# ogotoh/spaln

Hardware: AMD Instinct MI355X
Metric: GCUPS (DP cell updates/s), cDNA->genome spliced DP (higher is better)
Workload: dtype f32 (exact integers) / int32; 1 GPU; C2: 10k x 2 kb cDNA vs planted loci +-1 kb (windows ~12 kb), default band, Fwd2s1 _wip path: alignS_ng(ori=1, -Q0) = UDH sweep + slab tracebacks, SKL out; queries_per_gpu=10000, queries_total=10000, parallelism=1 rank(s), one per GPU, queries sharded, no collective on the data path

## Files before the change

### include/spdp.h

```cpp
#ifndef SPDP_H_
#define SPDP_H_

#include <stdint.h>
#include <stddef.h>

#ifdef __cplusplus
extern "C" {
#endif

#define SPDP_MAX_QUANT   8
#define SPDP_NEVSEL      (INT32_MIN / 16 * 7)
#define SPDP_END_OF_ULK  (INT32_MAX - 2)
#define SPDP_REF_NELEM   16

typedef struct SpdpScoring {
    int32_t mtx_dim;
    int32_t mtx[32 * 32];
    int32_t gop, gep;
    int32_t lgop, lgep;
    int32_t noll;
    int32_t spj;
    int32_t llmt;
    int32_t ipen;
    int32_t nquant;
// ... 129 lines not shown
typedef struct SpdpHspSource {
    void* user;
    int  (*units)(void* user, int32_t query, int32_t level, const int32_t span[8], const int32_t** flat, int32_t* n_flat);
    void (*release)(void* user, int32_t query, const int32_t* flat);
} SpdpHspSource;
int spdp_align_s_seeded(SpdpContext* ctx, const SpdpScoring* sc, const SpdpSeedParams* sp,
                        const SpdpProblem* probs, int n_probs, const SpdpJuxt* const* hsps, const int32_t* n_hsps,
                        const int32_t* lowest_level, const SpdpHspSource* src, SpdpAlignment* out);
int spdp_align_s_seeded_ori3(SpdpContext* ctx, const SpdpScoring* sc, const SpdpSeedParams* sp,
                             const SpdpProblem* fwd, const SpdpProblem* rev, int n_probs,
                             const SpdpJuxt* const* hsps, const int32_t* n_hsps, const int32_t* lowest_level,
                             const SpdpHspSource* src, SpdpAlignment* out, int32_t* orient);
int spdp_seeded_stats(const SpdpContext* ctx, int64_t* out, int n);
void spdp_rerun_stats(SpdpContext* ctx, int64_t* out, int reset);
void spdp_sweep_stats(SpdpContext* ctx, int64_t out[4], int reset);

int spdp_corner_list(const SpdpSkl* recs, int n, int m_unit, SpdpSkl* out);

typedef struct SpdpExon {
    int32_t left, right;
    int32_t rleft, rright;
    int32_t mch, mmc, gap, unp;
    int32_t mch5, mmc5, gap5, unp5;
    int32_t mch3, mmc3, gap3, unp3;
    int32_t phs;
    int32_t escr, iscr;
    int32_t sig3, sig5;
} SpdpExon;

typedef struct SpdpRescoreParams {
// ... 436 lines not shown
```

### spaln_amd/csrc/spdp_api.cpp

```cpp

#include <hip/hip_runtime.h>
#include <algorithm>
#include <cstdio>
#include <cstdlib>
#include <cstring>
#include <atomic>
#include <string>
#include <thread>
#include <vector>

#include "../../include/spdp.h"
#include "spdp_dev.h"
#include "spdp_internal.h"

static void stripe_rng(int a_left, int a_right, int b_left, int b_right, int sh, SpdpWindow* w)
{
    if (sh < 0) {
        int shorter = std::min(a_right - a_left, b_right - b_left);
        sh = -sh * shorter / 100;
    }
    w->up = b_right - a_right;
    w->lw = b_left - a_left;
    if (w->up < w->lw) std::swap(w->up, w->lw);
    w->up += sh;
// ... 117 lines not shown
        SpdpContext* l = spdp_create(ctx->device);
        if (!l) return nullptr;
        ctx->lanes.push_back(l);
    }
    return ctx->lanes[i - 1];
}

void spdp_destroy(SpdpContext* ctx)
{
    if (!ctx) return;
    for (SpdpContext* l : ctx->lanes) spdp_destroy(l);
    ctx->lanes.clear();
    (void) hipSetDevice(ctx->device);
    for (DevPool& p : ctx->pool) p.release();
    for (int k = 0; k < 3; ++k) if (ctx->stage_ptr[k]) (void) hipHostFree(ctx->stage_ptr[k]);
    (void) hipEventDestroy(ctx->ev0);
    (void) hipEventDestroy(ctx->ev1);
    (void) hipEventDestroy(ctx->ev2);
    (void) hipEventDestroy(ctx->ev3);
    if (ctx->stream2) (void) hipStreamDestroy(ctx->stream2);
    (void) hipStreamDestroy(ctx->stream);
    delete ctx;
}

void* SpdpContext::staging(int k, size_t bytes)
{
    if (bytes <= stage_cap[k]) return stage_ptr[k];
    if (stage_ptr[k]) (void) hipHostFree(stage_ptr[k]);
    stage_ptr[k] = nullptr; stage_cap[k] = 0;
    const size_t want = bytes + bytes / 8;
    if (hipHostMalloc(&stage_ptr[k], want, hipHostMallocDefault) != hipSuccess) { stage_ptr[k] = nullptr; return nullptr; }
    stage_cap[k] = want;
    return stage_ptr[k];
}

int spdp_upload_ring(SpdpContext* ctx, const std::vector<int64_t>& off, int64_t tot, int64_t grp_positions,
                     std::vector<StagedStream>& st, const std::function<void(int i, int64_t at)>& pack)
// ... 533 lines not shown
    case BY_ROWWAVE_UDH: HIPCHK(spdp_launch_rowwave_udh(&S, strm())); break;
    default:             HIPCHK(spdp_launch_rowwave(cut ? 2 : T.arg, &S, strm())); break;
    }
    HIPCHK(hipEventRecord(eve(), strm()));
    return 0;
}

int DevRun::launch_sweep()
{
    const RunTraits& T = traits();
    SweepArgs A;
    A.sc = (const DevScoring*) store->d_sc; A.probs = (const DevProblem*) d_probs; A.n_probs = n;
    A.a_codes = (const uint8_t*) store->d_a; A.cols = (const int2*) store->d_cols; A.bnd = (int*) d_bnd;
    A.tb = (uint8_t*) d_tb; A.imd = (int*) d_imd; A.res = (DevResult*) d_res; A.n_multi = n_multi;
    A.cross_g = cross_g; A.gprog = (int*) d_gprog;
    int grid = cross_g > 0 ? n * cross_g : n_multi + (n - n_multi + wpb - 1) / wpb;
    if (cross_g > 0 && getenv("SPDP_CROSS_TEST_SHORT")) --grid;
    HIPCHK(hipEventRecord(evb(), strm()));
    const int nq = std::max(1, std::min(store->sc.nquant, SPDP_MAX_QUANT));
    const int pen_cap = nq > 1 ? store->sc.qm_len[nq - 2] + 1 : 0;
    bool done = false;
    if (fp_ok && (T.kind != KIND_FORWARD || spdp_knob_on("SPDP_FP_FWD")) && !store->sc.local) {
        const hipError_t e = spdp_launch_sweep_fp(T.arg, 0, store->sc.spj ? 1 : 0, nq, pen_cap, store->sc.llmt, &A, grid, wpb, strm());
        if (e == hipSuccess) done = true;
        else if (e != hipErrorNotSupported) HIPCHK(e);
    }
    if (!done) HIPCHK(spdp_launch_sweep(T.arg, store->sc.local ? 1 : 0, nq, pen_cap, &A, grid, wpb, strm()));
    ++ctx->sweep_stats[done ? 0 : 1];
    if (cross_g > 0) ++ctx->sweep_stats[2];
    if (wpb == 16) ++ctx->sweep_stats[3];
// ... 15 lines not shown
    if (reset) ctx->rerun_stats[0] = ctx->rerun_stats[1] = 0;
    for (SpdpContext* l : ctx->lanes) {
        out[0] += l->rerun_stats[0]; out[1] += l->rerun_stats[1];
        if (reset) l->rerun_stats[0] = l->rerun_stats[1] = 0;
    }
}

extern "C" void spdp_sweep_stats(SpdpContext* ctx, int64_t* out, int reset)
{
    if (!ctx || !out) return;
    for (int k = 0; k < 4; ++k) {
        out[k] = reset ? ctx->sweep_stats[k].exchange(0) : ctx->sweep_stats[k].load();
        for (SpdpContext* l : ctx->lanes)
            out[k] += reset ? l->sweep_stats[k].exchange(0) : l->sweep_stats[k].load();
    }
}

int DevRun::sync()
{
    HIPCHK(hipStreamSynchronize(strm()));
    in_flight = false;
    if (cross_g > 0) {
        const size_t per = (size_t) cross_g * wpb + 2;
        std::vector<int> words(per * n);
        HIPCHK(spdp_copy_sync(words.data(), d_gprog, sizeof(int) * words.size(), hipMemcpyDeviceToHost, strm()));
        bool gave_up = false;
        for (int j = 0; j < n; ++j) gave_up = gave_up || words[per * j + per - 1] != 0;
        if (gave_up) {
            ++ctx->rerun_stats[0];
            if (getenv("SPDP_TRACE_RUNS")) fprintf(stderr, "[spdp run] a cross-CU group was not resident%s: launch repeated without the groups\n", side ? " (side stream, beside another launch)" : "");
// ... 274 lines not shown
```

### spaln_amd/csrc/spdp_host.cpp

```cpp

#include <algorithm>
#include <cmath>
#include <cstdlib>
#include <cstring>
#include <vector>
#include <chrono>
#include <condition_variable>
#include <cstdio>
#include <mutex>
#include <thread>

#include "spdp_internal.h"

namespace {

const int kEndOfUlk = SPDP_END_OF_ULK;
const float kCoefB = 2.0f;
const int kScalarRows = 8;

struct Rng { int al, ar, bl, br; uint8_t a_exgl, a_exgr, b_exgl, b_exgr; };

struct Job {
    int score = SPDP_NEVSEL;
    bool score_set = false;
    bool failed = false;
    bool edge = false;
    std::vector<SpdpSkl> rec;
// ... 101 lines not shown
    if (s.size() >= 2) {
        const int i = s[1].m - s[0].m, j = s[1].n - s[0].n;
        if ((p.a_exgl && !i) || (p.b_exgl && !j)) s.erase(s.begin());
    }
    if (s.size() >= 2) {
        const size_t k = s.size() - 1;
        const int i = s[k].m - s[k - 1].m, j = s[k].n - s[k - 1].n;
        if ((p.a_exgr && !i) || (p.b_exgr && !j)) s.pop_back();
    }
}

}
void trim_skl_of(std::vector<SpdpSkl>& s, const SpdpProblem& p) { trim_skl(s, p); }
namespace {

struct ChunkGate {
    std::mutex m;
    std::condition_variable cv;
    int state = 0;
    hipEvent_t ev = nullptr;
    void open(int st_) { { std::lock_guard<std::mutex> g(m); if (state == 0) state = st_; } cv.notify_all(); }
    int wait() { std::unique_lock<std::mutex> g(m); cv.wait(g, [&] { return state != 0; }); return state; }
};

struct Aligner {
    SpdpContext* ctx;
    const DevStore* st;
    const SpdpProblem* probs;
    int n;
    int base = 0;
    ChunkGate* gate_in = nullptr;
    ChunkGate* gate_out = nullptr;
    SpdpAlignment* out = nullptr;
    bool raw = false;
    const SpdpRequests* req = nullptr;
    int parent(int job) const { return req ? req->parents[base + job] : base + job; }
    std::vector<TbItem> ctbs;
    std::vector<Job> jobs;
// ... 144 lines not shown
            trcbk(u.job, cur, w, false);
        }
    }

    double t_mark = 0;
    bool timing = getenv("SPDP_TIMING") != nullptr;
    void lap(const char* what)
    {
        if (!timing) return;
        const double now = std::chrono::duration<double, std::milli>(
            std::chrono::steady_clock::now().time_since_epoch()).count();
        if (t_mark > 0) fprintf(stderr, "[spdp timing] %-28s %8.2f ms\n", what, now - t_mark);
        t_mark = now;
    }

    int run()
    {
        const int rc = run_chunk();
        if (gate_out) gate_out->open(2);
        if (!rc && out) for (int i = 0; i < n; ++i) finish(i, out + i);
        return rc;
    }

    int run_chunk()
    {
        const SpdpScoring& sc = st->sc;
        lap("start");
        jobs.assign(n, Job());
        for (int i = 0; i < n; ++i) {
            const SpdpProblem& p = probs[i];
            Rng r{p.a_left, p.a_right, p.b_left, p.b_right, p.a_exgl, p.a_exgr, p.b_exgl, p.b_exgr};
            SpdpWindow w;
            stripe_of(r, sc.sh, &w);
            if (req) {
// ... 29 lines not shown
                if (side.build(st, items, RUN_WIP_FORWARD) || side.launch()) return -1;
                lap("side fwd build+launch");
            }
            may_overlap = false;
            if (udh.empty()) continue;
            std::vector<RunItem> items;
            for (const UdhItem& u : udh) {
                items.push_back(run_item(parent(u.job), u.r, u.w, u.n_imd));
                items.back().imd_intvl = u.imd_intvl;
            }
            DevRun run(ctx);
            run.beside = !side_tbs.empty();
            const bool a0 = sc.scalar_engines == 1;
            if (run.build(st, items, a0 ? RUN_A0_UDH : (sc.scalar_engines == 2 ? RUN_A1_UDH : RUN_WIP_UDH))) return -1;
            lap("udh build");
            if (first_round && gate_in && gate_in->wait() == 1) HIPCHK(hipStreamWaitEvent(run.strm(), gate_in->ev, 0));
            if (run.launch()) return -1;
            if (first_round && gate_out) {
                HIPCHK(hipEventRecord(gate_out->ev, run.strm()));
                gate_out->open(1);
            }
            first_round = false;
            if (run.sync()) return -1;
            lap("udh launch+sync");
            kernel_ms += run.kernel_ms; kernel_cells += run.total_cells;
            stats[0] += run.kernel_ms; stats[1] += (double) run.total_cells; stats[2] += (double) items.size();
            stats[6] += 1;
            std::vector<int32_t> scores, cpos, ranges;
            std::vector<int32_t> edge;
            if (run.fetch_udh(scores, cpos, ranges, &edge)) return -1;
            std::vector<DevResult> ures;
            if (a0 && run.fetch_results(ures)) return -1;
            lap("udh fetch");
            const int stride = run.cpos_stride();
            for (size_t k = 0; k < udh.size(); ++k) {
// ... 142 lines not shown
        memcpy(out->skl + 1, s.data(), sizeof(SpdpSkl) * s.size());
    }
};

}

struct SpdpBatch {
    SpdpContext* ctx = nullptr;
    DevStore store;
    std::vector<SpdpProblem> probs;
    DevRun score;
    bool score_built = false;
    double stats[SPDP_N_STATS] = {0};
};

SpdpBatch* spdp_batch_upload(SpdpContext* ctx, const SpdpScoring* sc, const SpdpProblem* probs, int n)
{
    if (!ctx || n <= 0) return nullptr;
    SpdpBatch* b = new SpdpBatch();
    b->ctx = ctx;
    b->probs.assign(probs, probs + n);
    if (b->store.upload(ctx, sc, probs, n)) { delete b; return nullptr; }
    return b;
}

void spdp_batch_free(SpdpBatch* bt) { delete bt; }

int64_t spdp_batch_cells(const SpdpBatch* bt)
{
    if (!bt) return 0;
// ... 17 lines not shown
    }
    if (bt->score.launch() || bt->score.sync()) return -1;
    if (kernel_ms) *kernel_ms = bt->score.kernel_ms;
    if (scores) {
        std::vector<DevResult> r;
        if (bt->score.fetch_results(r)) return -1;
        for (size_t i = 0; i < r.size(); ++i) scores[i] = r[i].score;
    }
    return 0;
}

static int align_on_store(SpdpContext* ctx, const DevStore* st, const SpdpProblem* probs, int n,
                          SpdpAlignment* out, float* kernel_ms, int64_t* kernel_cells,
                          double* stats = nullptr, bool raw = false, const SpdpRequests* req = nullptr)
{
    int n_chunks = n >= 4096 ? 2 : 1;
    if (const char* e = getenv("SPDP_CHUNKS")) n_chunks = std::max(1, std::min(atoi(e), 8));
    n_chunks = std::min(n_chunks, std::max(1, n / 64));
    if (req) n_chunks = 1;
    std::vector<Aligner> al(n_chunks);
    std::vector<ChunkGate> gates(n_chunks);
    std::vector<int> rc(n_chunks, 0);
    for (int c = 0; c < n_chunks; ++c) {
        Aligner& a = al[c];
        a.ctx = spdp_lane(ctx, c);
        if (!a.ctx) { ctx->err = "cannot create a lane context"; return -1; }
        a.st = st;
        a.base = (int) ((int64_t) n * c / n_chunks);
        a.n = (int) ((int64_t) n * (c + 1) / n_chunks) - a.base;
        a.probs = probs + a.base;
        a.out = out ? out + a.base : nullptr;
        a.raw = raw;
        a.req = req;
        if (n_chunks > 1) {
            if (hipEventCreateWithFlags(&gates[c].ev, hipEventDisableTiming) != hipSuccess) {
                for (int k = 0; k < c; ++k) if (gates[k].ev) (void) hipEventDestroy(gates[k].ev);
                ctx->err = "hipEventCreate"; return -1;
            }
            a.gate_out = &gates[c];
            a.gate_in = c > 0 ? &gates[c - 1] : nullptr;
        }
    }
    std::vector<std::thread> workers;
    for (int c = 1; c < n_chunks; ++c)
        workers.emplace_back([&, c, lane_copies = t_lane_copies]() { (void) hipSetDevice(ctx->device); t_lane_copies = lane_copies; rc[c] = al[c].run(); });
    rc[0] = al[0].run();
    for (std::thread& t : workers) t.join();
    for (int c = 0; c < n_chunks; ++c) if (gates[c].ev) (void) hipEventDestroy(gates[c].ev);
    int unsupported = 0, overflowed = 0;
    float kms = 0.f; int64_t kc = 0;
    double st_sum[SPDP_N_STATS] = {0};
    for (int c = 0; c < n_chunks; ++c) {
        if (rc[c]) {
            if (c > 0) ctx->err = al[c].ctx->err;
            if (out) spdp_free_alignments(out, n);
            return -1;
        }
        kms += al[c].kernel_ms; kc += al[c].kernel_cells; unsupported += al[c].unsupported; overflowed += al[c].overflowed;
        for (int k = 0; k < SPDP_N_STATS; ++k) st_sum[k] += al[c].stats[k];
    }
    if (kernel_ms) *kernel_ms = kms;
    if (kernel_cells) *kernel_cells = kc;
    if (stats) memcpy(stats, st_sum, sizeof st_sum);
    if (unsupported) {
        ctx->err = "sub-problems with fewer than 8 query rows need the scalar exact engine: supply "
                   "SpdpScoring.intpen / t53 and SpdpProblem.cano5 / cano3 / dinc";
        return 1;
    }
    if (overflowed) {
// ... 72 lines not shown
```

### spaln_amd/csrc/spdp_internal.h

```cpp
#ifndef SPDP_INTERNAL_H_
#define SPDP_INTERNAL_H_

#include <hip/hip_runtime.h>
#include <stdint.h>
#include <algorithm>
#include <atomic>
#include <cstdlib>
#include <functional>
#include <string>
#include <vector>
#include "../../include/spdp.h"
#include "spdp_dev.h"
#include "spdp_hostcpus.h"

struct SweepArgs {
    const DevScoring* sc;
    const DevProblem* probs;
    int               n_probs;
    const uint8_t*    a_codes;
    const int2*       cols;
    int*              bnd;
    uint8_t*          tb;
    int*              imd;
    DevResult*        res;
    int               n_multi;
    int               cross_g;
    int*              gprog;
};

#define HIPCHK(call)                                                                     \
    do {                                                                                 \
        hipError_t e_ = (call);                                                          \
        if (e_ != hipSuccess) {                                                          \
            ctx->err = std::string(#call) + ": " + hipGetErrorString(e_);                \
            return -1;                                                                   \
        }                                                                                \
    } while (0)

struct WalkArgs {
    const DevProblem* probs;
    int               n_probs;
    const uint8_t*    tb;
    const DevResult*  res;
// ... 239 lines not shown
    DevPool pool[N_CTX_POOLS];
    int device = 0;
    int n_cu = 0;
    hipStream_t stream = nullptr;
    hipEvent_t ev0 = nullptr, ev1 = nullptr;
    hipStream_t stream2 = nullptr;
    hipEvent_t ev2 = nullptr, ev3 = nullptr;
    std::string name;
    std::string err;
    std::vector<SpdpContext*> lanes;
    int64_t seed_stats[12] = {0};
    const int32_t* seed_a_tlen = nullptr;
    std::vector<std::vector<SpdpPhaseMark>> seed_marks;
    int64_t rerun_stats[2] = {0, 0};
    std::atomic<int64_t> sweep_stats[4] = {};
    void*  stage_ptr[3] = {nullptr, nullptr, nullptr};
    size_t stage_cap[3] = {0, 0, 0};
    void*  staging(int k, size_t bytes);
};
SpdpContext* spdp_lane(SpdpContext* ctx, int i);

struct StagedStream {
    int    slot;
    void*  dev;
    size_t bytes;
    void*  host = nullptr;
};
int spdp_upload_ring(SpdpContext* ctx, const std::vector<int64_t>& off, int64_t tot, int64_t grp_positions,
                     std::vector<StagedStream>& st, const std::function<void(int i, int64_t at)>& pack);
int spdp_upload_cip(SpdpContext* ctx, int n, const std::function<const int32_t*(int i, size_t& len)>& row, std::vector<int32_t>& off,
// ... 75 lines not shown
    bool fp_ok = false;
    void* d_gprog = nullptr;
    bool cut = false;
    TilePipe pipe;
    int max_n_im = 0, max_skl = 0;
    int64_t total_cells = 0, tb_bytes = 0;
    std::vector<DevProblem> h_probs;
    std::vector<int> order;
    void *d_probs = nullptr, *d_bnd = nullptr, *d_tb = nullptr, *d_imd = nullptr, *d_res = nullptr,
         *d_skl = nullptr, *d_nskl = nullptr, *d_cpos = nullptr,
         *d_ranges = nullptr, *d_scores = nullptr;
    int skl_cap = 0;
    float kernel_ms = 0.f;
    bool side = false;
    bool in_flight = false;
    bool beside = false;
    hipStream_t strm() const { return side ? ctx->stream2 : ctx->stream; }
    hipEvent_t evb() const { return side ? ctx->ev2 : ctx->ev0; }
    hipEvent_t eve() const { return side ? ctx->ev3 : ctx->ev1; }
    explicit DevRun(SpdpContext* lane = nullptr) : use_ctx(lane) {}
    DevRun(const DevRun&) = delete;
    DevRun& operator=(const DevRun&) = delete;
    ~DevRun() { release(); }
    const RunTraits& traits() const { return RUN_TRAITS[flavour]; }
    DevPool& pool() const { return ctx->pool[side ? SIDE_POOL : traits().pool]; }
    void* take(int slot, size_t bytes);
    int cpos_stride() const { return 10 * (max_n_im + 1); }
    int build(const DevStore* st, const std::vector<RunItem>& items, RunFlavour flav);
    int check();
    int lay_out(const std::vector<RunItem>& items, ItemShare& tot);
// ... 30 lines not shown
```

### spaln_amd/csrc/spdp_kernels.hip

```cpp

#include <hip/hip_runtime.h>
#include <stdlib.h>
#include <stdint.h>
#include "spdp_dev.h"
#include "spdp_internal.h"
#include "spdp_wave.h"

enum { FL_SCORE = 0, FL_FORWARD = 1, FL_UDH = 2 };

enum { TB_DIAG = 1, TB_HORI = 2, TB_VERT = 8, TB_ACCR = 14, TB_NHOR = 16, TB_NVER = 32, TB_DONR = 128 };

#define END_OF_ULK (INT32_MAX - 2)

__device__ __forceinline__ int max3i(int a, int b, int c) { return max(max(a, b), c); }
template <bool B> struct BoolTag { static constexpr bool value = B; };

enum { NQ_FLAT = 0, NQ_TABLE = 1, NQ_CHAIN = 2 };
#define SPDP_PEN_TAB 2048

template <int FL, bool LOCAL, int NQM, int WPB, bool CROSS = false>
__global__ __launch_bounds__(WPB * 64) void spdp_sweep(SweepArgs A)
{
    constexpr int BW = (FL == FL_UDH) ? 4 : 2;
    __shared__ int s_mtx[32 * 32];
    __shared__ short s_pen[NQM == NQ_TABLE ? SPDP_PEN_TAB : 2];
    __shared__ int2 s_col[WPB][4][96];
    __shared__ int  s_feed[WPB][4][16 * BW];
    __shared__ int  s_out[WPB][4][16 * BW + BW];

    const DevScoring* __restrict__ sc = A.sc;
    for (int i = threadIdx.x; i < 32 * 32; i += blockDim.x) s_mtx[i] = sc->mtx[i];
    const int nquant = sc->nquant;
    const int pen_cap = (NQM == NQ_TABLE) ? sc->qm_len[nquant - 2] + 1 : 0;
    if constexpr (NQM == NQ_TABLE) {
        for (int h = threadIdx.x; h <= pen_cap; h += blockDim.x) {
            int pv = sc->qm_pen[0];
            for (int j = 1; j < nquant; ++j) if (h > sc->qm_len[j - 1]) pv = sc->qm_pen[j];
            s_pen[h] = (short) pv;
        }
    }
    __syncthreads();
    int ql[7], qp[7];
    #pragma unroll
    for (int j = 0; j < 7; ++j) {
// ... 462 lines not shown
            return;
        }
    }
    if constexpr (!LOCAL) {
        if (wpb == 16) {
            const dim3 blk(1024);
            switch (nqm) {
            case NQ_FLAT:  hipLaunchKernelGGL((spdp_sweep<FL, LOCAL, NQ_FLAT, 16>), grd, blk, 0, stream, A); break;
            case NQ_TABLE: hipLaunchKernelGGL((spdp_sweep<FL, LOCAL, NQ_TABLE, 16>), grd, blk, 0, stream, A); break;
            default:       hipLaunchKernelGGL((spdp_sweep<FL, LOCAL, NQ_CHAIN, 16>), grd, blk, 0, stream, A); break;
            }
            return;
        }
    }
    const dim3 blk(256);
    switch (nqm) {
    case NQ_FLAT:  hipLaunchKernelGGL((spdp_sweep<FL, LOCAL, NQ_FLAT, 4>), grd, blk, 0, stream, A); break;
    case NQ_TABLE: hipLaunchKernelGGL((spdp_sweep<FL, LOCAL, NQ_TABLE, 4>), grd, blk, 0, stream, A); break;
    default:       hipLaunchKernelGGL((spdp_sweep<FL, LOCAL, NQ_CHAIN, 4>), grd, blk, 0, stream, A); break;
    }
}

extern "C" hipError_t spdp_launch_sweep(int flavour, int local, int nquant, int pen_cap, const SweepArgs* args,
                                        int grid, int wpb, hipStream_t stream)
{
    SweepArgs A = *args;
    dim3 grd(grid);
    const int blk = (wpb == 16 && !local) ? 16 : 4;
    int nqm = nquant <= 1 ? NQ_FLAT : (pen_cap < SPDP_PEN_TAB ? NQ_TABLE : NQ_CHAIN);
    if (const char* e = getenv("SPDP_NQM")) { if (nqm != NQ_FLAT && atoi(e) == NQ_CHAIN) nqm = NQ_CHAIN; }
// ... 290 lines not shown
```

### spaln_amd/csrc/spdp_sweep_fp.hip

```cpp

#include <hip/hip_runtime.h>
#include <stdlib.h>
#include <stdint.h>
#include "spdp_dev.h"
#include "spdp_internal.h"
#include "spdp_wave.h"

namespace {

enum { FL_SCORE = 0, FL_FORWARD = 1, FL_UDH = 2 };

#define END_OF_ULK (INT32_MAX - 2)
#define SPDP_FPEN_TAB 992

constexpr float NEVF = (float) SPDP_NEV16;
constexpr float FLOORF = (float) SPDP_FLOOR16;
constexpr float BIGF = 4194304.f;

__device__ __forceinline__ float as_f(int x) { return __int_as_float(x); }
__device__ __forceinline__ int as_i(float x) { return __float_as_int(x); }

typedef __amdgpu_buffer_rsrc_t rsrc_t;
__device__ __forceinline__ rsrc_t bnd_rsrc(const int* base)
{
// ... 6 lines not shown
}
template <bool X> __device__ __forceinline__ int2 ldx_b2(rsrc_t r, const int* base, int64_t idx)
{
    if constexpr (X) { const v2i_t v = __builtin_amdgcn_raw_buffer_load_b64(r, (int) (idx * 4), 0, 16); return make_int2(v.x, v.y); }
    else return ld_nt2(base + idx);
}
template <bool B> struct BoolTag { static constexpr bool value = B; };
#ifndef SPDP_NO_PIN
#define SPDP_PIN_LOADS() __builtin_amdgcn_sched_barrier(0)
#else
#define SPDP_PIN_LOADS()
#endif

}

template <int FL, int WPB, bool CROSS, bool SPJ>
__global__ __launch_bounds__(WPB * 64) __attribute__((amdgpu_waves_per_eu(WPB == 4 && !CROSS ? 5 : 1))) void spdp_sweep_fp(SweepArgs A)
{
    constexpr bool UDH = FL == FL_UDH;
    constexpr bool FWD = FL == FL_FORWARD;
    enum { TB_DIAG = 1, TB_HORI = 2, TB_VERT = 8, TB_ACCR = 14, TB_NHOR = 16, TB_NVER = 32, TB_DONR = 128 };
    constexpr int BW = UDH ? 4 : 2;
    constexpr int RS = 80;
    __shared__ float  s_mtx[32 * 36];
    __shared__ int    s_perm[32];
    __shared__ float2 s_pen[SPDP_FPEN_TAB];
    __shared__ float2 s_sig[WPB][4][RS];
    __shared__ int    s_bof[WPB][4][RS];
    __shared__ int    s_io[WPB][4][16 * BW + BW];
    __shared__ int    s_prog_lds[WPB];

    const DevScoring* __restrict__ sc = A.sc;
    if (threadIdx.x < 32) {
        const int c = threadIdx.x;
        int below = 0;
        for (int x = 0; x < c; ++x) below += (x != 2 && x != 3 && x != 5 && x != 9);
        s_perm[c] = c == 2 ? 0 : c == 3 ? 1 : c == 5 ? 2 : c == 9 ? 3 : 4 + below;
    }
    __syncthreads();
    for (int i = threadIdx.x; i < 32 * 32; i += blockDim.x) s_mtx[s_perm[i >> 5] * 36 + s_perm[i & 31]] = (float) sc->mtx[i];
    const int nquant = sc->nquant, llmt = sc->llmt;
    const int pen_cap = max(nquant > 1 ? sc->qm_len[nquant - 2] + 1 : 0, llmt + 1);
    for (int h = threadIdx.x; SPJ && h <= pen_cap; h += blockDim.x) {
        int pv = sc->qm_pen[0];
        for (int j = 1; j < nquant; ++j) if (h > sc->qm_len[j - 1]) pv = sc->qm_pen[j];
        s_pen[h] = (h > llmt) ? make_float2(0.f, (float) pv) : make_float2(-BIGF, NEVF - FLOORF);
// ... 470 lines not shown
#undef BIDX
}

template <int FL, bool SPJ>
static hipError_t launch_fp(dim3 grd, int wpb, hipStream_t stream, const SweepArgs& A)
{
    if constexpr (FL == FL_UDH || FL == FL_FORWARD) {
        if (A.cross_g > 0) {
            SweepArgs Ac = A;
            void* kargs[] = {&Ac};
            const void* fn = wpb == 16 ? (const void*) spdp_sweep_fp<FL, 16, true, SPJ> : (const void*) spdp_sweep_fp<FL, 4, true, SPJ>;
            return hipLaunchCooperativeKernel(fn, grd, dim3(wpb == 16 ? 1024 : 256), kargs, 0, stream);
        }
    }
    static const int lds_pad = getenv("SPDP_LDS_PAD") ? atoi(getenv("SPDP_LDS_PAD")) : 0;
    if (wpb == 16) hipLaunchKernelGGL((spdp_sweep_fp<FL, 16, false, SPJ>), grd, dim3(1024), 0, stream, A);
    else           hipLaunchKernelGGL((spdp_sweep_fp<FL, 4, false, SPJ>), grd, dim3(256), lds_pad, stream, A);
    return hipGetLastError();
}

extern "C" int spdp_sweep_fp_serves(int local, int spj, int nquant, int pen_cap, int llmt)
{
    if (local) return 0;
    const int cap = nquant > 1 ? pen_cap : 0;
    return !(spj && (llmt < 1 || (cap > llmt + 1 ? cap : llmt + 1) >= SPDP_FPEN_TAB));
}

extern "C" hipError_t spdp_launch_sweep_fp(int flavour, int local, int spj, int nquant, int pen_cap, int llmt,
                                           const SweepArgs* args, int grid, int wpb, hipStream_t stream)
{
// ... 9 lines not shown
```

### spaln_amd/engine.py

```python
from __future__ import annotations

import ctypes as C
import os

import numpy as np

from . import abi

_HERE = os.path.dirname(os.path.abspath(__file__))
LIB_PATH = os.environ.get("SPDP_LIB") or os.path.join(_HERE, "libspdp_hip.so")

EXPORTS = [
    "spdp_create", "spdp_destroy", "spdp_last_error", "spdp_device_name", "spdp_stripe",
    "spdp_cells", "spdp_wip_scoreonly", "spdp_wip_forward", "spdp_wip_udh", "spdp_homscore_s",
    "spdp_align_s", "spdp_align_s_ori3", "spdp_free_alignments", "spdp_skl_rng_s", "spdp_skl_rng_h", "spdp_free_rescored", "spdp_scalar_forward", "spdp_scalar_scorealone", "spdp_scalar_udh", "spdp_batch_upload", "spdp_batch_free",
    "spdp_batch_cells", "spdp_batch_homscore", "spdp_batch_align", "spdp_batch_stats",
    "spdp_stripe31", "spdp_cells_h", "spdp_wip_forward_h", "spdp_wip_udh_h", "spdp_homscore_h", "spdp_align_h",
    "spdp_scalar_forward_h", "spdp_scalar_udh_h",
    "spdp_batch_upload_h", "spdp_batch_free_h", "spdp_batch_cells_h", "spdp_batch_align_h",
    "spdp_submit_align_s", "spdp_submit_homscore_s", "spdp_submit_align_h", "spdp_submit_homscore_h",
    "spdp_poll", "spdp_wait",
    "spdp_group_create", "spdp_group_destroy", "spdp_group_size", "spdp_group_last_error",
    "spdp_group_homscore_s", "spdp_group_align_s", "spdp_group_homscore_h", "spdp_group_align_h",
    "spdp_group_align_s_seeded", "spdp_group_align_h_seeded", "spdp_group_skl_rng_s", "spdp_group_skl_rng_h",
    "spdp_group_context", "spdp_group_blk_vote", "spdp_group_map_align_s",
    "spdp_align_s_seeded", "spdp_align_s_seeded_ori3", "spdp_seeded_stats",
    "spdp_blk_index_create", "spdp_blk_index_destroy", "spdp_blk_vote", "spdp_blk_vote_resident",
    "spdp_blk_search_opts_default", "spdp_blk_index_read", "spdp_blk_index_host_desc", "spdp_blk_index_host_free",
    "spdp_rerun_stats", "spdp_sweep_stats",
]


def load_library() -> C.CDLL:
    if not os.path.exists(LIB_PATH):
        raise RuntimeError(f"{LIB_PATH} not built: run `make -C spaln_amd/csrc` (or __graft_entry__.build())")
    lib = C.CDLL(LIB_PATH)
    lib.spdp_create.restype = C.c_void_p
    lib.spdp_create.argtypes = [C.c_int]
    lib.spdp_destroy.argtypes = [C.c_void_p]
    lib.spdp_last_error.restype = C.c_char_p
    lib.spdp_last_error.argtypes = [C.c_void_p]
    lib.spdp_device_name.argtypes = [C.c_void_p, C.c_char_p, C.c_int]
    lib.spdp_cells.restype = C.c_int64
    lib.spdp_splice_signals.argtypes = [C.c_void_p, C.c_void_p, C.c_void_p, C.c_int32, C.c_int32, C.c_int32,
# ... 46 lines not shown
    lib.spdp_lsp_s.argtypes = [C.c_void_p, C.c_void_p, C.c_void_p, C.c_int, C.c_void_p]
    lib.spdp_collector_create.restype = C.c_void_p
    lib.spdp_collector_create.argtypes = [C.c_void_p, C.c_void_p, C.c_int, C.c_int, C.c_int]
    lib.spdp_collector_destroy.argtypes = [C.c_void_p]
    lib.spdp_collector_align_s.argtypes = [C.c_void_p, C.c_void_p, C.c_void_p]
    lib.spdp_collector_last_error.restype = C.c_char_p
    lib.spdp_collector_last_error.argtypes = [C.c_void_p]
    lib.spdp_collector_stats.argtypes = [C.c_void_p, C.c_void_p, C.c_void_p, C.c_void_p]
    lib.spdp_group_create.restype = C.c_void_p
    lib.spdp_group_create.argtypes = [C.c_void_p, C.c_int]
    lib.spdp_group_destroy.argtypes = [C.c_void_p]
    lib.spdp_group_size.argtypes = [C.c_void_p]
    lib.spdp_group_last_error.restype = C.c_char_p
    lib.spdp_group_last_error.argtypes = [C.c_void_p]
    lib.spdp_group_last_shards.argtypes = [C.c_void_p, C.c_void_p, C.c_int]
    for f in ("spdp_rerun_stats", "spdp_sweep_stats"):
        getattr(lib, f).restype = None
        getattr(lib, f).argtypes = [C.c_void_p, C.c_void_p, C.c_int]
    lib.spdp_stripe.argtypes = [C.c_void_p, C.c_int, C.c_void_p]
    lib.spdp_cells.argtypes = [C.c_void_p, C.c_void_p]
    for f in ("spdp_group_homscore_s", "spdp_group_align_s", "spdp_group_homscore_h", "spdp_group_align_h"):
        getattr(lib, f).argtypes = [C.c_void_p, C.c_void_p, C.c_void_p, C.c_int, C.c_void_p]
    return lib


def exon_form(lib, eij, *, scr, gene_codes, protein, q_left, q_right, q_len, gmap, qmap, scale, aln_scale,
              q_many=1, q_sens=0, hsp_len=0, qname="qry", gname="win", header=False, gene_id=0):
    eij = np.ascontiguousarray(eij, dtype=np.int32).reshape(-1, 21)
    codes = np.ascontiguousarray(gene_codes, dtype=np.uint8)
    a = abi.ExonFormIn()
    a.eij, a.n_eij, a.scr = eij.ctypes.data, eij.shape[0], int(scr)
    a.gene_codes, a.gene_is_tron, a.qry_is_protein = codes.ctypes.data, int(bool(protein)), int(bool(protein))
    a.q_left, a.q_right, a.q_len, a.q_many, a.q_sens = int(q_left), int(q_right), int(q_len), int(q_many), int(q_sens)
# ... 187 lines not shown
    def device_name(self) -> str:
        buf = C.create_string_buffer(256)
        self.lib.spdp_device_name(self.ctx, buf, 256)
        return buf.value.decode()

    def rerun_stats(self, reset: bool = False) -> np.ndarray:
        out = np.zeros(2, dtype=np.int64)
        self.lib.spdp_rerun_stats(self.ctx, out.ctypes.data, int(bool(reset)))
        return out

    def sweep_stats(self, reset: bool = False) -> np.ndarray:
        out = np.zeros(4, dtype=np.int64)
        self.lib.spdp_sweep_stats(self.ctx, out.ctypes.data, int(bool(reset)))
        return out

    def splice_signals(self, model: abi.SignalModel, b_codes, left: int = 0, right=None) -> dict:
        b = np.ascontiguousarray(b_codes, dtype=np.uint8)
        n1 = b.size + 1
        out = dict(sig5=np.zeros(n1, np.int16), sig3=np.zeros(n1, np.int16), cano5=np.zeros(n1, np.uint8),
                   cano3=np.zeros(n1, np.uint8), dinc=np.zeros(n1, np.uint8))
        self._check(self.lib.spdp_splice_signals(self.ctx, C.addressof(model), b.ctypes.data, b.size, int(left),
                                                 int(b.size if right is None else right),
                                                 *(out[k].ctypes.data for k in ("sig5", "sig3", "cano5", "cano3", "dinc"))),
                    "spdp_splice_signals")
        return out

    def splice_signals_h(self, model: abi.SignalModelH, b_codes, left: int = 0, right=None) -> dict:
        b = np.ascontiguousarray(b_codes, dtype=np.uint8)
        b_len = b.size - 1
        n = b_len + 3
# ... 442 lines not shown
```

Measured before the change: 877.0 GCUPS.

## Plan cell-balanced chunks and signal kernel start to overlap chunk pipelines

Chunk boundaries are now chosen from per-problem DP cell counts (optionally geometric ratios) instead of equal problem counts, and more than two chunks rotate over two lane contexts. The first sweep kernel of a chunk writes a mapped host flag once all its blocks have started, so the next chunk can launch immediately instead of waiting on an event. The aim is to balance work between the overlapping lanes and shorten the idle gap between chunk launches. In exchange it adds host polling with sleeps, extra kernel template instantiations, and a per-call host pass to compute cell counts.

```diff
diff --git a/include/spdp.h b/include/spdp.h
--- a/include/spdp.h
+++ b/include/spdp.h
@@ -167,6 +167,8 @@
 int spdp_seeded_stats(const SpdpContext* ctx, int64_t* out, int n);
 void spdp_rerun_stats(SpdpContext* ctx, int64_t* out, int reset);
 void spdp_sweep_stats(SpdpContext* ctx, int64_t out[4], int reset);
+void spdp_chunk_stats(SpdpContext* ctx, int64_t out[6], int reset);
+int spdp_chunk_plan(const int64_t* cells, int n, int max_chunks, double ratio, int min_chunk, int* bounds);
 
 int spdp_corner_list(const SpdpSkl* recs, int n, int m_unit, SpdpSkl* out);
 
diff --git a/spaln_amd/csrc/spdp_api.cpp b/spaln_amd/csrc/spdp_api.cpp
--- a/spaln_amd/csrc/spdp_api.cpp
+++ b/spaln_amd/csrc/spdp_api.cpp
@@ -155,6 +155,8 @@
     (void) hipSetDevice(ctx->device);
     for (DevPool& p : ctx->pool) p.release();
     for (int k = 0; k < 3; ++k) if (ctx->stage_ptr[k]) (void) hipHostFree(ctx->stage_ptr[k]);
+    if (ctx->d_started) (void) hipFree(ctx->d_started);
+    if (ctx->sig_host) (void) hipHostFree(ctx->sig_host);
     (void) hipEventDestroy(ctx->ev0);
     (void) hipEventDestroy(ctx->ev1);
     (void) hipEventDestroy(ctx->ev2);
@@ -162,6 +164,19 @@
     if (ctx->stream2) (void) hipStreamDestroy(ctx->stream2);
     (void) hipStreamDestroy(ctx->stream);
     delete ctx;
+}
+
+int SpdpContext::start_signal()
+{
+    SpdpContext* ctx = this;
+    if (d_started && sig_host_dev) return 0;
+    if (!d_started) HIPCHK(hipMalloc((void**) &d_started, 256));
+    if (!sig_host) {
+        HIPCHK(hipHostMalloc((void**) &sig_host, 256, hipHostMallocMapped | hipHostMallocCoherent));
+        *sig_host = 0;
+    }
+    HIPCHK(hipHostGetDevicePointer((void**) &sig_host_dev, sig_host, 0));
+    return 0;
 }
 
 void* SpdpContext::staging(int k, size_t bytes)
@@ -725,6 +740,14 @@
     A.a_codes = (const uint8_t*) store->d_a; A.cols = (const int2*) store->d_cols; A.bnd = (int*) d_bnd;
     A.tb = (uint8_t*) d_tb; A.imd = (int*) d_imd; A.res = (DevResult*) d_res; A.n_multi = n_multi;
     A.cross_g = cross_g; A.gprog = (int*) d_gprog;
+    A.started = nullptr; A.started_host = nullptr;
+    signal_armed = signal_start && flavour == RUN_WIP_UDH && cross_g == 0 && wpb == 4 && !store->sc.local;
+    if (signal_armed) {
+        if (ctx->start_signal()) return -1;
+        HIPCHK(hipMemsetAsync(ctx->d_started, 0, sizeof(unsigned), strm()));
+        __atomic_store_n(ctx->sig_host, 0, __ATOMIC_RELEASE);
+        A.started = ctx->d_started; A.started_host = ctx->sig_host_dev;
+    }
     int grid = cross_g > 0 ? n * cross_g : n_multi + (n - n_multi + wpb - 1) / wpb;
     if (cross_g > 0 && getenv("SPDP_CROSS_TEST_SHORT")) --grid;
     HIPCHK(hipEventRecord(evb(), strm()));
@@ -770,6 +793,12 @@
         for (SpdpContext* l : ctx->lanes)
             out[k] += reset ? l->sweep_stats[k].exchange(0) : l->sweep_stats[k].load();
     }
+}
+
+extern "C" void spdp_chunk_stats(SpdpContext* ctx, int64_t* out, int reset)
+{
+    if (!ctx || !out) return;
+    for (int k = 0; k < 6; ++k) out[k] = reset ? ctx->chunk_stats[k].exchange(0) : ctx->chunk_stats[k].load();
 }
 
 int DevRun::sync()
diff --git a/spaln_amd/csrc/spdp_chunk_plan.h b/spaln_amd/csrc/spdp_chunk_plan.h
--- /dev/null
+++ b/spaln_amd/csrc/spdp_chunk_plan.h
@@ -0,0 +1,51 @@
+#ifndef SPDP_CHUNK_PLAN_H_
+#define SPDP_CHUNK_PLAN_H_
+#include <stdint.h>
+#include <algorithm>
+#include <vector>
+
+#define SPDP_CHUNK_LEAST 64
+
+static inline int spdp_chunk_plan_of(const int64_t* cells, int n, int max_chunks, double ratio, int min_chunk, int* bounds)
+{
+    bounds[0] = 0; bounds[1] = std::max(n, 0);
+    if (n <= 0 || max_chunks <= 1) return 1;
+    const int least = std::max(SPDP_CHUNK_LEAST, min_chunk);
+    if (!(ratio > 0.) || ratio > 1.) ratio = 1.;
+    std::vector<int64_t> cum((size_t) n + 1, 0);
+    int64_t biggest = 1;
+    for (int i = 0; i < n; ++i) {
+        const int64_t c = std::max<int64_t>(cells[i], 1);
+        cum[i + 1] = cum[i] + c;
+        biggest = std::max(biggest, c);
+    }
+    const double total = (double) cum[n];
+    auto held = [&](int c) { return cum[bounds[c + 1]] - cum[bounds[c]]; };
+    for (int k = std::min(max_chunks, n / least); k >= 2; --k) {
+        double wsum = 0., w = 1.;
+        for (int c = 0; c < k; ++c) { wsum += w; w *= ratio; }
+        double acc = 0.;
+        w = 1.;
+        for (int c = 0; c + 1 < k; ++c) {
+            acc += w; w *= ratio;
+            const double target = total * acc / wsum;
+            const int lo = bounds[c] + least, hi = n - (k - 1 - c) * least;
+            int i = lo;
+            while (i < hi && (double) cum[i] + 0.5 < target) ++i;
+            bounds[c + 1] = i;
+        }
+        bounds[k] = n;
+        for (bool moved = true; moved; ) {
+            moved = false;
+            for (int c = 0; c + 1 < k; ++c)
+                while (held(c + 1) > held(c) && bounds[c + 2] - bounds[c + 1] > least) { ++bounds[c + 1]; moved = true; }
+        }
+        bool ok = true;
+        for (int c = 0; c + 1 < k; ++c) ok = ok && held(c + 1) <= held(c) + biggest;
+        if (ok) return k;
+    }
+    bounds[1] = n;
+    return 1;
+}
+
+#endif
diff --git a/spaln_amd/csrc/spdp_host.cpp b/spaln_amd/csrc/spdp_host.cpp
--- a/spaln_amd/csrc/spdp_host.cpp
+++ b/spaln_amd/csrc/spdp_host.cpp
@@ -11,6 +11,7 @@
 #include <thread>
 
 #include "spdp_internal.h"
+#include "spdp_chunk_plan.h"
 
 namespace {
 
@@ -142,14 +143,27 @@
 void trim_skl_of(std::vector<SpdpSkl>& s, const SpdpProblem& p) { trim_skl(s, p); }
 namespace {
 
+enum GateState : int { GATE_SHUT = 0, GATE_EVENT = 1, GATE_NONE = 2, GATE_LAUNCH_NOW = 3 };
 struct ChunkGate {
     std::mutex m;
     std::condition_variable cv;
-    int state = 0;
+    int state = GATE_SHUT;
+    int opened = 0;
     hipEvent_t ev = nullptr;
-    void open(int st_) { { std::lock_guard<std::mutex> g(m); if (state == 0) state = st_; } cv.notify_all(); }
-    int wait() { std::unique_lock<std::mutex> g(m); cv.wait(g, [&] { return state != 0; }); return state; }
+    void open(int st_)
+    {
+        {
+            std::lock_guard<std::mutex> g(m);
+            if (state == GATE_SHUT || st_ != GATE_NONE) ++opened;
+            if (state == GATE_SHUT) state = st_;
+        }
+        cv.notify_all();
+    }
+    int wait() { std::unique_lock<std::mutex> g(m); cv.wait(g, [&] { return state != GATE_SHUT; }); return state; }
 };
+
+constexpr int    kDefaultChunks = 2;
+constexpr double kDefaultChunkRatio = 1.0;
 
 struct Aligner {
     SpdpContext* ctx;
@@ -324,10 +338,21 @@
         t_mark = now;
     }
 
+    static bool started(const DevRun& run)
+    {
+        if (!run.signal_armed) return false;
+        const int* word = run.ctx->sig_host;
+        for (unsigned look = 0; !__atomic_load_n(word, __ATOMIC_ACQUIRE); ++look) {
+            if (look % 16 == 15 && hipEventQuery(run.eve()) != hipErrorNotReady) return __atomic_load_n(word, __ATOMIC_ACQUIRE) != 0;
+            std::this_thread::sleep_for(std::chrono::microseconds(30));
+        }
+        return true;
+    }
+
     int run()
     {
         const int rc = run_chunk();
-        if (gate_out) gate_out->open(2);
+        if (gate_out) gate_out->open(GATE_NONE);
         if (!rc && out) for (int i = 0; i < n; ++i) finish(i, out + i);
         return rc;
     }
@@ -387,11 +412,12 @@
             const bool a0 = sc.scalar_engines == 1;
             if (run.build(st, items, a0 ? RUN_A0_UDH : (sc.scalar_engines == 2 ? RUN_A1_UDH : RUN_WIP_UDH))) return -1;
             lap("udh build");
-            if (first_round && gate_in && gate_in->wait() == 1) HIPCHK(hipStreamWaitEvent(run.strm(), gate_in->ev, 0));
+            if (first_round && gate_in && gate_in->wait() == GATE_EVENT) HIPCHK(hipStreamWaitEvent(run.strm(), gate_in->ev, 0));
+            run.signal_start = first_round && gate_out;
             if (run.launch()) return -1;
             if (first_round && gate_out) {
                 HIPCHK(hipEventRecord(gate_out->ev, run.strm()));
-                gate_out->open(1);
+                gate_out->open(started(run) ? GATE_LAUNCH_NOW : GATE_EVENT);
             }
             first_round = false;
             if (run.sync()) return -1;
@@ -564,6 +590,12 @@
     double stats[SPDP_N_STATS] = {0};
 };
 
+int spdp_chunk_plan(const int64_t* cells, int n, int max_chunks, double ratio, int min_chunk, int* bounds)
+{
+    if (!cells || !bounds) return 0;
+    return spdp_chunk_plan_of(cells, n, std::max(1, max_chunks), ratio, min_chunk, bounds);
+}
+
 SpdpBatch* spdp_batch_upload(SpdpContext* ctx, const SpdpScoring* sc, const SpdpProblem* probs, int n)
 {
     if (!ctx || n <= 0) return nullptr;
@@ -611,45 +643,76 @@
                           SpdpAlignment* out, float* kernel_ms, int64_t* kernel_cells,
                           double* stats = nullptr, bool raw = false, const SpdpRequests* req = nullptr)
 {
-    int n_chunks = n >= 4096 ? 2 : 1;
-    if (const char* e = getenv("SPDP_CHUNKS")) n_chunks = std::max(1, std::min(atoi(e), 8));
-    n_chunks = std::min(n_chunks, std::max(1, n / 64));
-    if (req) n_chunks = 1;
+    int max_chunks = n >= 4096 ? kDefaultChunks : 1, min_chunk = 5 * std::max(1, ctx->n_cu);
+    double ratio = kDefaultChunkRatio;
+    if (const char* e = getenv("SPDP_CHUNKS")) { max_chunks = std::max(1, std::min(atoi(e), 8)); min_chunk = SPDP_CHUNK_LEAST; }
+    if (const char* e = getenv("SPDP_CHUNK_RATIO")) ratio = atof(e);
+    if (req) max_chunks = 1;
+    std::vector<int> bounds((size_t) max_chunks + 1, 0);
+    int n_chunks = 1;
+    bounds[1] = n;
+    if (max_chunks > 1 && n >= 2 * SPDP_CHUNK_LEAST) {
+        std::vector<int64_t> cells(n);
+        const auto t0 = std::chrono::steady_clock::now();
+        for (int i = 0; i < n; ++i) {
+            SpdpWindow w;
+            spdp_stripe(&probs[i], st->sc.sh, &w);
+            cells[i] = spdp_cells(&probs[i], &w);
+        }
+        n_chunks = spdp_chunk_plan_of(cells.data(), n, max_chunks, ratio, min_chunk, bounds.data());
+        if (getenv("SPDP_TIMING"))
+            fprintf(stderr, "[spdp timing] %-28s %8.2f ms  (%d chunks)\n", "chunk plan (cells + bounds)",
+                    std::chrono::duration<double, std::milli>(std::chrono::steady_clock::now() - t0).count(), n_chunks);
+    }
+    const int n_lanes = std::min(n_chunks, 2);
     std::vector<Aligner> al(n_chunks);
     std::vector<ChunkGate> gates(n_chunks);
     std::vector<int> rc(n_chunks, 0);
     for (int c = 0; c < n_chunks; ++c) {
         Aligner& a = al[c];
-        a.ctx = spdp_lane(ctx, c);
+        a.ctx = spdp_lane(ctx, c % 2);
         if (!a.ctx) { ctx->err = "cannot create a lane context"; return -1; }
         a.st = st;
-        a.base = (int) ((int64_t) n * c / n_chunks);
-        a.n = (int) ((int64_t) n * (c + 1) / n_chunks) - a.base;
+        a.base = bounds[c];
+        a.n = bounds[c + 1] - bounds[c];
         a.probs = probs + a.base;
         a.out = out ? out + a.base : nullptr;
         a.raw = raw;
         a.req = req;
-        if (n_chunks > 1) {
+        if (c + 1 < n_chunks) {
             if (hipEventCreateWithFlags(&gates[c].ev, hipEventDisableTiming) != hipSuccess) {
                 for (int k = 0; k < c; ++k) if (gates[k].ev) (void) hipEventDestroy(gates[k].ev);
                 ctx->err = "hipEventCreate"; return -1;
             }
             a.gate_out = &gates[c];
-            a.gate_in = c > 0 ? &gates[c - 1] : nullptr;
-        }
-    }
+        }
+        a.gate_in = c > 0 ? &gates[c - 1] : nullptr;
+    }
+    auto run_lane = [&](int lane) {
+        bool failed = false;
+        for (int c = lane; c < n_chunks; c += n_lanes) {
+            if (!failed) failed = (rc[c] = al[c].run()) != 0;
+            else { rc[c] = -1; if (al[c].gate_out) al[c].gate_out->open(GATE_NONE); }
+        }
+    };
     std::vector<std::thread> workers;
-    for (int c = 1; c < n_chunks; ++c)
-        workers.emplace_back([&, c, lane_copies = t_lane_copies]() { (void) hipSetDevice(ctx->device); t_lane_copies = lane_copies; rc[c] = al[c].run(); });
-    rc[0] = al[0].run();
+    for (int l = 1; l < n_lanes; ++l)
+        workers.emplace_back([&, l, lane_copies = t_lane_copies]() { (void) hipSetDevice(ctx->device); t_lane_copies = lane_copies; run_lane(l); });
+    run_lane(0);
     for (std::thread& t : workers) t.join();
+    ctx->chunk_stats[0] += 1; ctx->chunk_stats[1] += n_chunks;
+    for (int c = 0; c + 1 < n_chunks; ++c) {
+        const int how = gates[c].state;
+        ctx->chunk_stats[how == GATE_LAUNCH_NOW ? 2 : how == GATE_EVENT ? 3 : 4] += 1;
+        if (gates[c].opened == 1) ctx->chunk_stats[5] += 1;
+    }
     for (int c = 0; c < n_chunks; ++c) if (gates[c].ev) (void) hipEventDestroy(gates[c].ev);
     int unsupported = 0, overflowed = 0;
     float kms = 0.f; int64_t kc = 0;
     double st_sum[SPDP_N_STATS] = {0};
     for (int c = 0; c < n_chunks; ++c) {
         if (rc[c]) {
-            if (c > 0) ctx->err = al[c].ctx->err;
+            if (al[c].ctx != ctx) ctx->err = al[c].ctx->err;
             if (out) spdp_free_alignments(out, n);
             return -1;
         }
diff --git a/spaln_amd/csrc/spdp_internal.h b/spaln_amd/csrc/spdp_internal.h
--- a/spaln_amd/csrc/spdp_internal.h
+++ b/spaln_amd/csrc/spdp_internal.h
@@ -26,7 +26,19 @@
     int               n_multi;
     int               cross_g;
     int*              gprog;
-};
+    unsigned*         started;
+    int*              started_host;
+};
+
+#if defined(__HIPCC__)
+__device__ __forceinline__ void spdp_signal_started(const SweepArgs& A)
+{
+    if (A.started != nullptr && threadIdx.x == 0) {
+        const unsigned before = __hip_atomic_fetch_add(A.started, 1u, __ATOMIC_RELAXED, __HIP_MEMORY_SCOPE_AGENT);
+        if (before + 1 == gridDim.x) __hip_atomic_store(A.started_host, 1, __ATOMIC_RELAXED, __HIP_MEMORY_SCOPE_SYSTEM);
+    }
+}
+#endif
 
 #define HIPCHK(call)                                                                     \
     do {                                                                                 \
@@ -296,6 +308,11 @@
     std::vector<std::vector<SpdpPhaseMark>> seed_marks;
     int64_t rerun_stats[2] = {0, 0};
     std::atomic<int64_t> sweep_stats[4] = {};
+    unsigned* d_started = nullptr;
+    int*      sig_host = nullptr;
+    int*      sig_host_dev = nullptr;
+    int       start_signal();
+    std::atomic<int64_t> chunk_stats[6] = {};
     void*  stage_ptr[3] = {nullptr, nullptr, nullptr};
     size_t stage_cap[3] = {0, 0, 0};
     void*  staging(int k, size_t bytes);
@@ -401,6 +418,8 @@
     float kernel_ms = 0.f;
     bool side = false;
     bool in_flight = false;
+    bool signal_start = false;
+    bool signal_armed = false;
     bool beside = false;
     hipStream_t strm() const { return side ? ctx->stream2 : ctx->stream; }
     hipEvent_t evb() const { return side ? ctx->ev2 : ctx->ev0; }
diff --git a/spaln_amd/csrc/spdp_kernels.hip b/spaln_amd/csrc/spdp_kernels.hip
--- a/spaln_amd/csrc/spdp_kernels.hip
+++ b/spaln_amd/csrc/spdp_kernels.hip
@@ -18,7 +18,7 @@
 enum { NQ_FLAT = 0, NQ_TABLE = 1, NQ_CHAIN = 2 };
 #define SPDP_PEN_TAB 2048
 
-template <int FL, bool LOCAL, int NQM, int WPB, bool CROSS = false>
+template <int FL, bool LOCAL, int NQM, int WPB, bool CROSS = false, bool SIG = false>
 __global__ __launch_bounds__(WPB * 64) void spdp_sweep(SweepArgs A)
 {
     constexpr int BW = (FL == FL_UDH) ? 4 : 2;
@@ -28,6 +28,7 @@
     __shared__ int  s_feed[WPB][4][16 * BW];
     __shared__ int  s_out[WPB][4][16 * BW + BW];
 
+    if constexpr (SIG) spdp_signal_started(A);
     const DevScoring* __restrict__ sc = A.sc;
     for (int i = threadIdx.x; i < 32 * 32; i += blockDim.x) s_mtx[i] = sc->mtx[i];
     const int nquant = sc->nquant;
@@ -520,6 +521,16 @@
         }
     }
     const dim3 blk(256);
+    if constexpr (!LOCAL && FL == FL_UDH) {
+        if (A.started != nullptr) {
+            switch (nqm) {
+            case NQ_FLAT:  hipLaunchKernelGGL((spdp_sweep<FL, LOCAL, NQ_FLAT, 4, false, true>), grd, blk, 0, stream, A); break;
+            case NQ_TABLE: hipLaunchKernelGGL((spdp_sweep<FL, LOCAL, NQ_TABLE, 4, false, true>), grd, blk, 0, stream, A); break;
+            default:       hipLaunchKernelGGL((spdp_sweep<FL, LOCAL, NQ_CHAIN, 4, false, true>), grd, blk, 0, stream, A); break;
+            }
+            return;
+        }
+    }
     switch (nqm) {
     case NQ_FLAT:  hipLaunchKernelGGL((spdp_sweep<FL, LOCAL, NQ_FLAT, 4>), grd, blk, 0, stream, A); break;
     case NQ_TABLE: hipLaunchKernelGGL((spdp_sweep<FL, LOCAL, NQ_TABLE, 4>), grd, blk, 0, stream, A); break;
diff --git a/spaln_amd/csrc/spdp_sweep_fp.hip b/spaln_amd/csrc/spdp_sweep_fp.hip
--- a/spaln_amd/csrc/spdp_sweep_fp.hip
+++ b/spaln_amd/csrc/spdp_sweep_fp.hip
@@ -44,7 +44,7 @@
 
 }
 
-template <int FL, int WPB, bool CROSS, bool SPJ>
+template <int FL, int WPB, bool CROSS, bool SPJ, bool SIG = false>
 __global__ __launch_bounds__(WPB * 64) __attribute__((amdgpu_waves_per_eu(WPB == 4 && !CROSS ? 5 : 1))) void spdp_sweep_fp(SweepArgs A)
 {
     constexpr bool UDH = FL == FL_UDH;
@@ -60,6 +60,7 @@
     __shared__ int    s_io[WPB][4][16 * BW + BW];
     __shared__ int    s_prog_lds[WPB];
 
+    if constexpr (SIG) spdp_signal_started(A);
     const DevScoring* __restrict__ sc = A.sc;
     if (threadIdx.x < 32) {
         const int c = threadIdx.x;
@@ -560,6 +561,12 @@
         }
     }
     static const int lds_pad = getenv("SPDP_LDS_PAD") ? atoi(getenv("SPDP_LDS_PAD")) : 0;
+    if constexpr (FL == FL_UDH) {
+        if (wpb != 16 && A.started != nullptr) {
+            hipLaunchKernelGGL((spdp_sweep_fp<FL, 4, false, SPJ, true>), grd, dim3(256), lds_pad, stream, A);
+            return hipGetLastError();
+        }
+    }
     if (wpb == 16) hipLaunchKernelGGL((spdp_sweep_fp<FL, 16, false, SPJ>), grd, dim3(1024), 0, stream, A);
     else           hipLaunchKernelGGL((spdp_sweep_fp<FL, 4, false, SPJ>), grd, dim3(256), lds_pad, stream, A);
     return hipGetLastError();
diff --git a/spaln_amd/engine.py b/spaln_amd/engine.py
--- a/spaln_amd/engine.py
+++ b/spaln_amd/engine.py
@@ -27,7 +27,7 @@
     "spdp_align_s_seeded", "spdp_align_s_seeded_ori3", "spdp_seeded_stats",
     "spdp_blk_index_create", "spdp_blk_index_destroy", "spdp_blk_vote", "spdp_blk_vote_resident",
     "spdp_blk_search_opts_default", "spdp_blk_index_read", "spdp_blk_index_host_desc", "spdp_blk_index_host_free",
-    "spdp_rerun_stats", "spdp_sweep_stats",
+    "spdp_rerun_stats", "spdp_sweep_stats", "spdp_chunk_stats", "spdp_chunk_plan",
 ]
 
 
@@ -104,9 +104,11 @@
     lib.spdp_group_last_error.restype = C.c_char_p
     lib.spdp_group_last_error.argtypes = [C.c_void_p]
     lib.spdp_group_last_shards.argtypes = [C.c_void_p, C.c_void_p, C.c_int]
-    for f in ("spdp_rerun_stats", "spdp_sweep_stats"):
+    for f in ("spdp_rerun_stats", "spdp_sweep_stats", "spdp_chunk_stats"):
         getattr(lib, f).restype = None
         getattr(lib, f).argtypes = [C.c_void_p, C.c_void_p, C.c_int]
+    lib.spdp_chunk_plan.restype = C.c_int
+    lib.spdp_chunk_plan.argtypes = [C.c_void_p, C.c_int, C.c_int, C.c_double, C.c_int, C.c_void_p]
     lib.spdp_stripe.argtypes = [C.c_void_p, C.c_int, C.c_void_p]
     lib.spdp_cells.argtypes = [C.c_void_p, C.c_void_p]
     for f in ("spdp_group_homscore_s", "spdp_group_align_s", "spdp_group_homscore_h", "spdp_group_align_h"):
@@ -324,6 +326,11 @@
         self.lib.spdp_sweep_stats(self.ctx, out.ctypes.data, int(bool(reset)))
         return out
 
+    def chunk_stats(self, reset: bool = False) -> np.ndarray:
+        out = np.zeros(6, dtype=np.int64)
+        self.lib.spdp_chunk_stats(self.ctx, out.ctypes.data, int(bool(reset)))
+        return out
+
     def splice_signals(self, model: abi.SignalModel, b_codes, left: int = 0, right=None) -> dict:
         b = np.ascontiguousarray(b_codes, dtype=np.uint8)
         n1 = b.size + 1
```

Result: faster. 896.0 GCUPS, median of 6 (+2.2%).
